# blasif/cocons

Measured on AMD Instinct MI355X. Metric: -2loglik evals/sec (dense cov_rns + Cholesky/solve/log-det, fp64) at n=10000, higher is better.
Workload: dtype f64

## Files before the change

### cocons_amd/csrc/chol.hip

```cpp
#include <hip/hip_runtime.h>
#include <limits.h>
#include <stdlib.h>
#include <string.h>
#include <algorithm>
#include <atomic>
#include <vector>
#include "kernels.h"

namespace cocons {

typedef double d4 __attribute__((ext_vector_type(4)));

#define MFMA64(a, b, c) __builtin_amdgcn_mfma_f64_16x16x4f64((a), (b), (c), 0, 0, 0)
#define MFMA64_NEGA(a, b, c) __builtin_amdgcn_mfma_f64_16x16x4f64((a), (b), (c), 0, 0, 1)
#define LDS_T __attribute__((address_space(3)))

__device__ __forceinline__ void blk_mma(d4 &acc, const d4 &P, const d4 &Q)
{
    acc = MFMA64(Q[0], P[0], acc);
    acc = MFMA64(Q[1], P[1], acc);
    acc = MFMA64(Q[2], P[2], acc);
    acc = MFMA64(Q[3], P[3], acc);
}

__device__ __forceinline__ d4 lds_blk(const double *blk, int lane)
{
    d4 v;
    int o = (lane >> 4) * 16 + (lane & 15);
    v[0] = blk[o];
    v[1] = blk[o + 64];
    v[2] = blk[o + 128];
    v[3] = blk[o + 192];
    return v;
}

__device__ __forceinline__ void lds_blk_store(double *blk, int lane, const d4 &v)
{
    int o = (lane >> 4) * 16 + (lane & 15);
    blk[o] = v[0];
    blk[o + 64] = v[1];
    blk[o + 128] = v[2];
    blk[o + 192] = v[3];
}

__device__ __forceinline__ d4 glb_blk(const double *A, size_t lda, int row0, int col0, int lane)
{
    const double *p = A + (size_t)(row0 + (lane & 15)) + (size_t)(col0 + (lane >> 4)) * lda;
    d4 v;
    v[0] = p[0];
    v[1] = p[4 * lda];
    v[2] = p[8 * lda];
    v[3] = p[12 * lda];
    return v;
}

__device__ __forceinline__ void glb_blk_store(double *A, size_t lda, int row0, int col0, int lane, const d4 &v)
{
    double *p = A + (size_t)(row0 + (lane & 15)) + (size_t)(col0 + (lane >> 4)) * lda;
    p[0] = v[0];
    p[4 * lda] = v[1];
    p[8 * lda] = v[2];
    p[12 * lda] = v[3];
}

__device__ __forceinline__ void store_wt(double *p, double v)
{
    __hip_atomic_store((unsigned long long *)p, (unsigned long long)__double_as_longlong(v), __ATOMIC_RELAXED,
                       __HIP_MEMORY_SCOPE_AGENT);
}

__device__ __forceinline__ double load_wt(const double *p)
{
    return __longlong_as_double((long long)__hip_atomic_load((const unsigned long long *)p, __ATOMIC_RELAXED,
                                                             __HIP_MEMORY_SCOPE_AGENT));
}

__device__ __forceinline__ d4 glb_blk_wt(const double *A, size_t lda, int row0, int col0, int lane)
{
    const double *p = A + (size_t)(row0 + (lane & 15)) + (size_t)(col0 + (lane >> 4)) * lda;
    d4 v;
    v[0] = load_wt(p);
    v[1] = load_wt(p + 4 * lda);
    v[2] = load_wt(p + 8 * lda);
    v[3] = load_wt(p + 12 * lda);
    return v;
}

__device__ __forceinline__ void glb_blk_store_wt(double *A, size_t lda, int row0, int col0, int lane, const d4 &v)
{
    double *p = A + (size_t)(row0 + (lane & 15)) + (size_t)(col0 + (lane >> 4)) * lda;
    store_wt(p, v[0]);
    store_wt(p + 4 * lda, v[1]);
    store_wt(p + 8 * lda, v[2]);
    store_wt(p + 12 * lda, v[3]);
}

__device__ __forceinline__ double rdlane(double v, int lane)
{
    int lo = __builtin_amdgcn_readlane(__double2loint(v), lane);
    int hi = __builtin_amdgcn_readlane(__double2hiint(v), lane);
    return __hiloint2double(hi, lo);
}

__device__ __forceinline__ void rsqrt_pivot(double a, double &l, double &r)
{
    const double y0 = __builtin_amdgcn_rsq(a);
    const double s0 = a * y0;
    const double t = fma(-s0, y0, 1.0);
    const double y = fma(y0 * t, fma(t, 0.375, 0.5), y0);
    double s = a * y;
    s = fma(fma(-s, s, a), 0.5 * y, s);
    l = s;
    r = y;
}

__device__ __forceinline__ double sel_lower4(int c, int k, double v00, double v10, double v11, double v20,
                                             double v21, double v22, double v30, double v31, double v32, double v33)
{
    double r0 = v00;
    double r1 = (k == 0) ? v10 : v11;
    double r2 = (k == 0) ? v20 : ((k == 1) ? v21 : v22);
    double r3 = (k == 0) ? v30 : ((k == 1) ? v31 : ((k == 2) ? v32 : v33));
    double r = (c == 0) ? r0 : ((c == 1) ? r1 : ((c == 2) ? r2 : r3));
    return (k <= c) ? r : 0.0;
}

template <int S>
__device__ __forceinline__ void potrf16_step(d4 &D, double (&Q)[4], int lane, int &fail)
{
    const int m = lane & 15, k = lane >> 4;
    const double ds = D[S];
    double a00 = rdlane(ds, 4 * S + 0), a10 = rdlane(ds, 4 * S + 1), a20 = rdlane(ds, 4 * S + 2),
           a30 = rdlane(ds, 4 * S + 3);
    double a11 = rdlane(ds, 4 * S + 1 + 16), a21 = rdlane(ds, 4 * S + 2 + 16), a31 = rdlane(ds, 4 * S + 3 + 16);
    double a22 = rdlane(ds, 4 * S + 2 + 32), a32 = rdlane(ds, 4 * S + 3 + 32);
    double a33 = rdlane(ds, 4 * S + 3 + 48);
    double l00, r0;
    rsqrt_pivot(a00, l00, r0);
    double l10 = a10 * r0, l20 = a20 * r0, l30 = a30 * r0;
    double t11 = fma(-l10, l10, a11);
    double l11, r1;
    rsqrt_pivot(t11, l11, r1);
    double l21 = fma(-l20, l10, a21) * r1, l31 = fma(-l30, l10, a31) * r1;
    double t22 = fma(-l21, l21, fma(-l20, l20, a22));
    double l22, r2;
    rsqrt_pivot(t22, l22, r2);
    double l32 = fma(-l31, l21, fma(-l30, l20, a32)) * r2;
    double t33 = fma(-l32, l32, fma(-l31, l31, fma(-l30, l30, a33)));
    double l33, r3;
    rsqrt_pivot(t33, l33, r3);
    if (__builtin_amdgcn_ballot_w64(!(t33 > 0.0)) != 0ull && fail == 0)
        fail = 4 * S + (!(a00 > 0.0) ? 1 : (!(t11 > 0.0) ? 2 : (!(t22 > 0.0) ? 3 : 4)));
    double m00 = r0, m11 = r1, m22 = r2, m33 = r3;
    double m10 = -(l10 * m00) * r1;
// ... 982 lines not shown
        }
    }
#pragma unroll
    for (int j = 0; j < 8; ++j) glb_blk_store(A, lda, rs, c0 + 16 * j, lane, B0[j]);
    if (split) return;
    if (tid == 0) ok = wait_ge<false>(xrw, 1u, abort_word, abort_code(ABORT_INPANEL, (unsigned)(c0 / TILE))) ? 1 : 0;
    asm volatile("s_waitcnt vmcnt(0)" ::: "memory");
    __syncthreads();
    if (!ok) return;
    {
        const int i = tid & 15, k = tid >> 4;
        const double *Xg = A + (size_t)(c1 + i) + (size_t)(c0 + k) * lda;
        double st[2][16];
#pragma unroll
        for (int b = 0; b < 16; ++b) st[0][b] = load_wt(Xg + (size_t)(16 * (b >> 3)) + (size_t)(16 * (b & 7)) * lda);
#pragma unroll
        for (int r = 0; r < 4; ++r) {
            if (r + 1 < 4) {
#pragma unroll
                for (int b = 0; b < 16; ++b) {
                    const int bb = 16 * (r + 1) + b;
                    st[(r + 1) & 1][b] = load_wt(Xg + (size_t)(16 * (bb >> 3)) + (size_t)(16 * (bb & 7)) * lda);
                }
            }
#pragma unroll
            for (int b = 0; b < 16; ++b) XS[(16 * r + b) * 256 + k * 16 + i] = st[r & 1][b];
        }
        __syncthreads();
#pragma unroll
        for (int jj = 0; jj < 8; ++jj) {
            d4 acc = {0.0, 0.0, 0.0, 0.0};
#pragma unroll
            for (int kb = 0; kb < 8; ++kb) {
                d4 Xb = lds_blk(XS + (jj * 8 + kb) * 256, lane);
                blk_mma(acc, B0[kb], Xb);
            }
            B1[jj] = B1[jj] - acc;
        }
    }
    __syncthreads();
    {
        const double *mb = mb1;
        double v9[3][9];
        MBOX_FETCH256V(0, v9[0])
        MBOX_FETCH256V(1, v9[1])
#pragma unroll
        for (int j = 0; j < 8; ++j) {
            double *LS = SM + (j & 1) * (9 * 256);
            MBOX_COMPLETE256V(j, v9[j % 3], abort_word, abort_code(ABORT_PANEL, (unsigned)(c1 / TILE)))
#pragma unroll
            for (int i = 0; i < 9; ++i)
                if (i <= 8 - j) LS[tid + 256 * i] = v9[j % 3][i];
            __syncthreads();
            if (!ok) return;
            if (j + 2 < 8) MBOX_FETCH256V(j + 2, v9[(j + 2) % 3])
            d4 L = lds_blk(LS, lane);
            double Q[4];
#pragma unroll
            for (int s = 0; s < 4; ++s) Q[s] = LS[(8 - j) * 256 + s * 64 + lane];
            trsm16(B1[j], L, Q);
            if (pub) mbox_store(sp + (size_t)(8 + j) * 1024, lane, B1[j]);
            d4 NX = -B1[j];
#pragma unroll
            for (int jj = j + 1; jj < 8; ++jj) {
                d4 Lb = lds_blk(LS + (jj - j) * 256, lane);
                blk_mma(B1[jj], NX, Lb);
            }
        }
    }
#pragma unroll
    for (int j = 0; j < 8; ++j) glb_blk_store(A, lda, rs, c1 + 16 * j, lane, B1[j]);
}

__global__ void __launch_bounds__(64)
engine_gate_kernel(unsigned *alive, unsigned *abort_word, unsigned code, unsigned long long ticks, unsigned nhelp,
                   unsigned *raise_in)
{
    if (threadIdx.x == 0) {
        bool ok = wait_ge<false>(alive, 1u, abort_word, code, ticks);
        if (ok && nhelp) ok = wait_ge<false>(alive + 2, nhelp, abort_word, code + 1u, ticks);
        if (ok && raise_in) {
            __hip_atomic_store(raise_in, 3u, __ATOMIC_RELAXED, __HIP_MEMORY_SCOPE_AGENT);
            __hip_atomic_store(raise_in + 1, 7u, __ATOMIC_RELAXED, __HIP_MEMORY_SCOPE_AGENT);
        }
    }
}

__global__ void __launch_bounds__(256)
trsm_tile_kernel(double *A, size_t lda, int c0, int r0, const double *qin, unsigned *wait_word, unsigned *abort_word,
                 int nb1, int e0, int own_world, int own_rank, int own_group)
{
    __shared__ double SL[36 * 256];
    __shared__ double QS[8 * 256];
    __shared__ int ok;
    const int tid = threadIdx.x, lane = tid & 63, wave = tid >> 6;
    if (own_world > 1) {
        const int row = (int)blockIdx.x < nb1 ? r0 + 64 * (int)blockIdx.x : e0 + 64 * ((int)blockIdx.x - nb1);
        if (((row / (2 * TILE) / own_group) % own_world) != own_rank) return;
    }
    if (wait_word) {
        if (tid == 0) ok = wait_ge<false>(wait_word, 1u, abort_word, abort_code(ABORT_PANEL, (unsigned)(c0 / TILE))) ? 1 : 0;
        asm volatile("s_waitcnt vmcnt(0)" ::: "memory");
        __syncthreads();
        if (!ok) return;
        fetch_factor_tile<true>(A, lda, c0, qin, SL, QS, tid);
    } else
        fetch_factor_tile<false>(A, lda, c0, qin, SL, QS, tid);
    const int bx = blockIdx.x;
    const int rs = (bx < nb1 ? r0 + 64 * bx : e0 + 64 * (bx - nb1)) + 16 * wave;
    d4 B[8];
#pragma unroll
    for (int j = 0; j < 8; ++j) B[j] = glb_blk(A, lda, rs, c0 + 16 * j, lane);
    __syncthreads();
#pragma unroll
    for (int j = 0; j < 8; ++j) {
        d4 L = lds_blk(SL + (j * (j + 1) / 2 + j) * 256, lane);
        double Q[4];
#pragma unroll
        for (int s = 0; s < 4; ++s) Q[s] = QS[j * 256 + s * 64 + lane];
        trsm16(B[j], L, Q);
        d4 NX = -B[j];
#pragma unroll
        for (int jj = j + 1; jj < 8; ++jj) {
            d4 Lb = lds_blk(SL + (jj * (jj + 1) / 2 + j) * 256, lane);
            blk_mma(B[jj], NX, Lb);
        }
    }
#pragma unroll
    for (int j = 0; j < 8; ++j) glb_blk_store(A, lda, rs, c0 + 16 * j, lane, B[j]);
}


struct UpdArgs {
    double *C; size_t ldc;
    const double *P; size_t ldp;
    int K;
    int ti0, tj0, lower_only;
    int H, W;
    unsigned *sig; int sig_tile;
    unsigned *wait_word, *abort_word;
    int ptiles, world, rank;
    const int *pmap;
    int skip_lo, skip_hi;
    unsigned *queue; unsigned ntiles;
    int Hb, ext0;
    int c_wt;
    int skew, kblk;
};

template <int TM, int KC, int ROLE, int NW = 4>
__global__ void __launch_bounds__(64 * NW, 8)
update_kernel(UpdArgs a)
{
    constexpr int LDT = TM + 16;
    constexpr int WY = NW / 2;
    constexpr int NB = TM / 32;
    constexpr int NBY = TM / WY / 16;
    constexpr int TPC = 64 * NW / KC;
    constexpr int RPT = TM / TPC;
    __shared__ double sI[2][KC * LDT];
    __shared__ double sJ[2][KC * LDT];
    unsigned *share = (unsigned *)&sI[0][TM];
    const int tid = threadIdx.x;
    const int wave_s = __builtin_amdgcn_readfirstlane(tid >> 6);
    if (a.wait_word) {
        if (tid == 0) *share = wait_ge(a.wait_word, 1u, a.abort_word, abort_code(ABORT_INPANEL, (unsigned)a.tj0)) ? 1u : 0u;
        asm volatile("s_waitcnt vmcnt(0)" ::: "memory");
        __syncthreads();
        const unsigned ok = *share;
        __syncthreads();
        if (!ok) return;
    }

    else if (a.abort_word) {
        if (tid == 0) *share = __hip_atomic_load(a.abort_word, __ATOMIC_RELAXED, __HIP_MEMORY_SCOPE_AGENT);
        __syncthreads();
        const unsigned ab = *share;
        __syncthreads();
        if (ab) return;
    }

    const int nch = a.K / KC;
    typedef double d2 __attribute__((ext_vector_type(2)));

    unsigned L = blockIdx.x;
    for (;;) {
        int lane;
        asm volatile("v_mbcnt_lo_u32_b32 %0, -1, 0\n\tv_mbcnt_hi_u32_b32 %0, -1, %0" : "=v"(lane));
        const int wave = wave_s, t2 = 64 * wave + lane;
        const int wi = wave & 1, wj = wave >> 1;
        const int kc = t2 / TPC, rg = (t2 % TPC) * RPT;
        const int ro = (lane >> 4) * LDT + (lane & 15);
        int ti, tj;
        if (a.lower_only) {
            int lo = 0, hi = a.W - 1;
            while (lo < hi) {
                const int mid = (lo + hi + 1) >> 1;
                if (mid * a.H - mid * (mid - 1) / 2 <= (int)L) lo = mid; else hi = mid - 1;
            }
            const int j = lo;
            const int til = j + ((int)L - (j * a.H - j * (j - 1) / 2));
            tj = a.tj0 + j;
            ti = til < a.Hb ? a.tj0 + til : a.ext0 + (til - a.Hb);
        } else {
            const int til = blockIdx.x;
            ti = til < a.Hb ? a.ti0 + til : a.ext0 + (til - a.Hb);
            tj = a.tj0 + blockIdx.y;
        }
        if (a.world > 1 && ((ti * TM / (2 * TILE) / a.ptiles) % a.world) != a.rank) return;
        if (ti >= a.skip_lo && ti < a.skip_hi && tj >= a.skip_lo && tj < a.skip_hi) {
            if (!a.queue) return;
            if (t2 == 0) *share = gridDim.x + __hip_atomic_fetch_add(a.queue, 1u, __ATOMIC_RELAXED, __HIP_MEMORY_SCOPE_AGENT);
            __syncthreads();
            L = (unsigned)__builtin_amdgcn_readfirstlane((int)*share);
            __syncthreads();
            if (L >= a.ntiles) break;
            continue;
        }
        const int sig_Ti = (ti * TM) / TILE - a.sig_tile, sig_Tj = (tj * TM) / TILE - a.sig_tile;
        const bool sig_wg = a.sig != nullptr && sig_Ti >= 0 && sig_Ti <= 1 && sig_Tj >= 0 && sig_Tj <= sig_Ti;
        const bool wt_wg = sig_wg || a.c_wt;
        if (sig_wg) __builtin_amdgcn_s_setprio(3); else __builtin_amdgcn_s_setprio(0);

        int rowI_P = ti * TM, rowJ_P = tj * TM, rowI_C = ti * TM;
        if (a.pmap) { rowI_P = a.pmap[ti]; rowJ_P = a.pmap[tj]; }
        if (a.skew) {
            const bool ext = ti >= a.ext0;
            const int under = a.skew * TILE + (ti - a.ext0) * TM;
            rowI_P = ext ? under : ti * TM - TILE * a.kblk;
            rowJ_P = tj * TM - TILE * a.kblk;
            rowI_C = ext ? under : ti * TM - TILE * ((tj * TM) / TILE);
        }
        const double *gI = a.P + (size_t)(rowI_P + rg) + (size_t)kc * a.ldp;
        const double *gJ = a.P + (size_t)(rowJ_P + rg) + (size_t)kc * a.ldp;
        d2 stI[RPT / 2], stJ[RPT / 2];

        double *Cb = a.C + (size_t)(rowI_C + (TM / 2) * wi) + (size_t)(tj * TM + (TM / WY) * wj) * a.ldc;
        const unsigned ldcb = 8u * (unsigned)a.ldc;
        const unsigned cvo = 8u * (unsigned)(lane & 15) + (unsigned)(lane >> 4) * ldcb;
        d4 acc[NB][NBY];
#pragma unroll
        for (int x = 0; x < NB; ++x)
#pragma unroll
            for (int y = 0; y < NBY; ++y) acc[x][y] = (d4){0.0, 0.0, 0.0, 0.0};

#pragma unroll
        for (int v = 0; v < RPT / 2; ++v) {
            stI[v] = *(const d2 *)(gI + 2 * v);
            stJ[v] = *(const d2 *)(gJ + 2 * v);
        }
#pragma unroll
        for (int v = 0; v < RPT / 2; ++v) {
            *(d2 *)(&sI[0][kc * LDT + rg + 2 * v]) = stI[v];
            *(d2 *)(&sJ[0][kc * LDT + rg + 2 * v]) = stJ[v];
        }
        __syncthreads();

        for (int ch = 0; ch < nch; ++ch) {
            const int cur = ch & 1;
            if (ch + 1 < nch) {
                const double *pI = gI + (size_t)(ch + 1) * KC * a.ldp;
                const double *pJ = gJ + (size_t)(ch + 1) * KC * a.ldp;
#pragma unroll
                for (int v = 0; v < RPT / 2; ++v) {
                    stI[v] = *(const d2 *)(pI + 2 * v);
                    stJ[v] = *(const d2 *)(pJ + 2 * v);
                }
            }
            const double *bI = &sI[cur][ro + (TM / 2) * wi];
            const double *bJ = &sJ[cur][ro + (TM / WY) * wj];
#pragma unroll
            for (int s = 0; s < KC / 4; ++s) {
                double pi_[NB], pj_[NBY];
#pragma unroll
                for (int x = 0; x < NB; ++x) pi_[x] = bI[s * 4 * LDT + 16 * x];
#pragma unroll
                for (int y = 0; y < NBY; ++y) pj_[y] = bJ[s * 4 * LDT + 16 * y];
#pragma unroll
                for (int x = 0; x < NB; ++x)
#pragma unroll
                    for (int y = 0; y < NBY; ++y) acc[x][y] = MFMA64(pj_[y], pi_[x], acc[x][y]);
            }
            if (ch + 1 < nch) {
#pragma unroll
                for (int v = 0; v < RPT / 2; ++v) {
                    *(d2 *)(&sI[cur ^ 1][kc * LDT + rg + 2 * v]) = stI[v];
                    *(d2 *)(&sJ[cur ^ 1][kc * LDT + rg + 2 * v]) = stJ[v];
                }
            }
            __syncthreads();
        }
        unsigned Lnext = 0;
        if (a.queue && t2 == 0)
            Lnext = gridDim.x + __hip_atomic_fetch_add(a.queue, 1u, __ATOMIC_RELAXED, __HIP_MEMORY_SCOPE_AGENT);
        unsigned cve = cvo;
        asm volatile("" : "+v"(cve));
#pragma unroll
        for (int x = 0; x < NB; ++x)
#pragma unroll
            for (int y = 0; y < NBY; ++y) {
                d4 cv;
#pragma unroll
                for (int r = 0; r < 4; ++r) {
                    const double *cp = (const double *)((const char *)(Cb + 16 * x) + (cve + (unsigned)(16 * y + 4 * r) * ldcb));
                    cv[r] = a.c_wt ? load_wt(cp) : *cp;
                }
                cv -= acc[x][y];
                if (wt_wg) {
#pragma unroll
                    for (int r = 0; r < 4; ++r)
                        store_wt((double *)((char *)(Cb + 16 * x) + (cve + (unsigned)(16 * y + 4 * r) * ldcb)), cv[r]);
                } else {
#pragma unroll
                    for (int r = 0; r < 4; ++r)
                        *(double *)((char *)(Cb + 16 * x) + (cve + (unsigned)(16 * y + 4 * r) * ldcb)) = cv[r];
                }
            }
        if (wt_wg) {
            asm volatile("s_waitcnt vmcnt(0)" ::: "memory");
            __syncthreads();
            if (t2 == 0 && sig_wg) signal_add(a.sig + a.sig_tile + sig_Ti);
        }
        if (!a.queue) break;
        if (t2 == 0) *share = Lnext;
        __syncthreads();
        L = (unsigned)__builtin_amdgcn_readfirstlane((int)*share);
        if (L >= a.ntiles) break;
    }
}

struct DagStep {
    unsigned base;
    unsigned near;
    unsigned tpos, nT;
    int H, W;
    int tj0;
    int k0, K;
    int nstrip, two;
    int need;
    int nd_next;
    int split;
    unsigned p2, p3;
};

struct DagArgs {
    double *A; size_t lda;
    double *P;
    const double *Wt;
    const DagStep *steps; int nsteps;
    unsigned ntasks;
    unsigned *queue;
    unsigned *tdone;
    unsigned *pdone; int pstride;
    unsigned *pall;
    double *partbuf;
    unsigned *dcount;
    unsigned *sig;
    unsigned *out, *xr;
    unsigned *abort_word;
    const unsigned *alive;
    unsigned xcc_quota;
    unsigned *hw;
    unsigned long long *trace;
    const unsigned *ftab;
    unsigned xcd_g;
    unsigned *xcnt;
};

constexpr unsigned DAG_XCD_LAG = 64u;
__device__ __forceinline__ unsigned dag_position(unsigned c, unsigned cls, unsigned g)
{
    return ((c >> g) << (g + 3u)) | (cls << g) | (c & ((1u << g) - 1u));
}

__device__ __forceinline__ bool dag_wait(const DagArgs &a, unsigned *word, unsigned need, unsigned code, unsigned L)
{
    const unsigned long long t0 = __builtin_amdgcn_s_memrealtime();
    for (unsigned it = 0;; ++it) {
        const unsigned v = poll_word(word, it);
        if (v >= need) break;
        if (__hip_atomic_load(a.abort_word, __ATOMIC_RELAXED, __HIP_MEMORY_SCOPE_AGENT) != 0u) return false;
        if (it > (unsigned)(ENGINE_TIMEOUT_TICKS / 100ull) ||
            ((it & 1023u) == 1023u && __builtin_amdgcn_s_memrealtime() - t0 > WALL_BACKSTOP_TICKS)) {
            if (__hip_atomic_exchange(a.abort_word, code, __ATOMIC_RELAXED, __HIP_MEMORY_SCOPE_AGENT) == 0u) {
                unsigned *d = a.queue + 8;
                d[0] = L; d[1] = code; d[2] = (unsigned)(word - a.queue); d[3] = need; d[4] = v;
                d[5] = (unsigned)(__builtin_amdgcn_s_memrealtime() - t0);
                d[6] = it;
            }
            return false;
        }
        __builtin_amdgcn_s_sleep(16);
    }
    __builtin_amdgcn_fence(__ATOMIC_ACQUIRE, "wavefront");
    return true;
}

__global__ void __launch_bounds__(256, 8)
dag_kernel(DagArgs a)
{
    constexpr int TM = 64, KC = 4, RING = 4, STG = 2 * KC * TM;
    __shared__ double smem[RING * STG + 2];
    unsigned *share = (unsigned *)&smem[RING * STG];
    const int tid = threadIdx.x;
    const int wave_s = __builtin_amdgcn_readfirstlane(tid >> 6);
    const DagStep *__restrict__ steps = a.steps;
    const unsigned ldab = 8u * (unsigned)a.lda;
    int known = 0;
    const unsigned myx = (hw_where() >> 28) & 7u;
    const bool loyal = ((blockIdx.x >> 3) & 1u) == 0u;
    if (tid == 0) {
        bool take = true;
        if (a.xcc_quota) {
            const unsigned c = __hip_atomic_load(a.alive + 16 + myx, __ATOMIC_RELAXED, __HIP_MEMORY_SCOPE_AGENT);
            if (c) {
                const unsigned less = 7u * (c - 1u);
                const unsigned quota = a.xcc_quota > less + 8u ? a.xcc_quota - less : 8u;
                take = __hip_atomic_fetch_add(a.queue + 16 + myx, 1u, __ATOMIC_RELAXED, __HIP_MEMORY_SCOPE_AGENT) < quota;
            }
        }
        unsigned first = 0xffffffffu;
        if (take) {
            if (a.xcd_g) first = dag_position(__hip_atomic_fetch_add(a.xcnt + 32u * myx, 1u, __ATOMIC_RELAXED, __HIP_MEMORY_SCOPE_AGENT), myx, a.xcd_g);
            else first = __hip_atomic_fetch_add(a.queue, 1u, __ATOMIC_RELAXED, __HIP_MEMORY_SCOPE_AGENT);
        }
        share[1] = first;
        share[2] = 0u;
    }
    __syncthreads();
    unsigned L = (unsigned)__builtin_amdgcn_readfirstlane((int)share[1]);
    __syncthreads();
    if (L >= a.ntasks) return;
    for (;;) {
        int lo = 0, hi = a.nsteps - 1;
        while (lo < hi) {
            const int mid = (lo + hi + 1) >> 1;
            if (steps[mid].base <= L) lo = mid; else hi = mid - 1;
        }
        const int s = lo;
        const DagStep st = steps[s];
        const unsigned q = L - st.base;
        if (a.trace && tid == 0) {
            a.trace[4 * (size_t)L] = __builtin_amdgcn_s_memrealtime();
            if (a.hw) a.hw[2 * (size_t)L] = hw_where();
// ... 497 lines not shown
__global__ void __launch_bounds__(256)
gather_rows_kernel(const double *Y, int ldy, const int *pos, int n, int ncol, double *out, int ldo)
{
    const int i = blockIdx.x * blockDim.x + threadIdx.x;
    if (i >= n) return;
    const int k = pos[i];
    for (int s = blockIdx.y; s < ncol; s += gridDim.y) out[(size_t)i + (size_t)s * ldo] = Y[(size_t)k + (size_t)s * ldy];
}

void launch_gather_rows(const double *Y, int ldy, const int *pos, int n, int ncol, double *out, int ldo, hipStream_t s)
{
    if (n <= 0 || ncol <= 0) return;
    const int gy = ncol < 64 ? ncol : 64;
    hipLaunchKernelGGL(gather_rows_kernel, dim3((n + 255) / 256, gy), dim3(256), 0, s, Y, ldy, pos, n, ncol, out, ldo);
}

static void set_dynamic_lds_once(const void *kernel, size_t bytes, std::atomic<unsigned long long> &done_mask)
{
    int dev = 0;
    (void)hipGetDevice(&dev);
    if (dev >= 0 && dev < 64 && ((done_mask.load(std::memory_order_relaxed) >> dev) & 1ull)) return;
    (void)hipFuncSetAttribute(kernel, hipFuncAttributeMaxDynamicSharedMemorySize, (int)bytes);
    if (dev >= 0 && dev < 64) done_mask.fetch_or(1ull << dev, std::memory_order_relaxed);
}

void launch_potrf_tile(double *A, size_t lda, int c0, double *dinv, int *info, hipStream_t s)
{
    const size_t shm = (36 + 1) * 256 * sizeof(double);
    static std::atomic<unsigned long long> attr_done{0};
    set_dynamic_lds_once((const void *)potrf_tile_kernel, shm, attr_done);
    hipLaunchKernelGGL(potrf_tile_kernel, dim3(1), dim3(512), shm, s, A, lda, c0, dinv, info);
}

__global__ void __launch_bounds__(64)
raise_word_kernel(unsigned *word)
{
    if (threadIdx.x == 0) __hip_atomic_store(word, 1u, __ATOMIC_RELAXED, __HIP_MEMORY_SCOPE_AGENT);
}

void launch_raise_word(unsigned *word, hipStream_t s) { hipLaunchKernelGGL(raise_word_kernel, dim3(1), dim3(64), 0, s, word); }

int streams_run_concurrently(hipStream_t first, hipStream_t second, unsigned *words)
{
    if (hipMemsetAsync(words, 0, 2 * sizeof(unsigned), second) != hipSuccess) return -1;
    if (hipStreamSynchronize(second) != hipSuccess) return -1;
    hipLaunchKernelGGL(engine_gate_kernel, dim3(1), dim3(64), 0, first, words, words + 1, 1u, 200000ull, 0u, (unsigned *)nullptr);
    hipLaunchKernelGGL(raise_word_kernel, dim3(1), dim3(64), 0, second, words);
    unsigned h[2] = {0, 0};
    if (hipStreamSynchronize(first) != hipSuccess || hipStreamSynchronize(second) != hipSuccess) return -1;
    if (hipMemcpyAsync(h, words, sizeof h, hipMemcpyDeviceToHost, second) != hipSuccess) return -1;
    if (hipStreamSynchronize(second) != hipSuccess) return -1;
    return h[1] == 0 ? 1 : 0;
}

void launch_engine_gate(unsigned *alive, unsigned *abort_word, hipStream_t s, bool last_tile, bool patient, int nhelp,
                        unsigned *raise_in)
{
    hipLaunchKernelGGL(engine_gate_kernel, dim3(1), dim3(64), 0, s, alive, abort_word, last_tile ? ABORT_LAST_TILE : ABORT_GATE,
                       last_tile ? ENGINE_TIMEOUT_TICKS : (patient ? 10 * GATE_TIMEOUT_TICKS : GATE_TIMEOUT_TICKS),
                       (unsigned)(last_tile || nhelp < 0 ? 0 : nhelp), last_tile ? nullptr : raise_in);
}

static size_t engine_lds_bytes()
{
    static size_t shm = 0;
    if (!shm) {
        shm = 150 * 1024;
        const char *x = getenv("COCONS_ENGINE_LDS");
        if (x && (size_t)atol(x) >= shm) shm = (size_t)atol(x);
    }
    return shm;
}

void launch_potrf_engine(double *A, size_t lda, int t0, int nt, double *dinv, int *info,
                         unsigned *in, unsigned *out, unsigned *xr, unsigned *abort_word, unsigned *alive, hipStream_t s,
                         double *wbuf, double *pbuf, int dag_until, unsigned long long *trace, double *mbox, int in_wait_ms)
{
    EngineArgs e;
    e.A = A; e.lda = lda; e.t0 = t0; e.nt = nt; e.dinv = dinv; e.info = info;
    e.in = in; e.out = out; e.xr = xr; e.abort_word = abort_word; e.alive = alive;
    e.wbuf = wbuf; e.pbuf = pbuf; e.dag_until = dag_until; e.trace = trace;
    e.in_ticks = in_wait_ms > 0 ? 100000ull * (unsigned long long)in_wait_ms : HOST_PACED_TICKS;
    e.mbox = mbox;
    e.partner = mbox ? 8 : 0;
    const int grid = e.partner ? e.partner + 1 : 1;
    const size_t shm = engine_lds_bytes();
    if (wbuf && pbuf) {
        static std::atomic<unsigned long long> attr_done{0};
        set_dynamic_lds_once((const void *)potrf_engine_kernel<true>, shm, attr_done);
        hipLaunchKernelGGL(potrf_engine_kernel<true>, dim3(grid), dim3(512), shm, s, e);
    } else {
        static std::atomic<unsigned long long> attr_done{0};
        set_dynamic_lds_once((const void *)potrf_engine_kernel<false>, shm, attr_done);
        hipLaunchKernelGGL(potrf_engine_kernel<false>, dim3(grid), dim3(512), shm, s, e);
    }
}

void launch_trsm_tile(double *A, size_t lda, int c0, int r0, int r1, const double *dinv, hipStream_t s,
                      unsigned *wait_word, unsigned *abort_word, int band_r1, int ext_r0, int own_world, int own_rank,
                      int own_group)
{
    int nb1 = ((band_r1 >= 0 ? band_r1 : r1) - r0) / 64, nb2 = band_r1 >= 0 ? (r1 - ext_r0) / 64 : 0;
    if (nb1 < 0) nb1 = 0;
    if (nb2 < 0) nb2 = 0;
    if (nb1 + nb2 <= 0) return;
    hipLaunchKernelGGL(trsm_tile_kernel, dim3(nb1 + nb2), dim3(256), 0, s, A, lda, c0, r0, dinv, wait_word, abort_word,
                       nb1, ext_r0, own_world, own_rank, own_group < 1 ? 1 : own_group);
}

void launch_potrf_follow(double *A, size_t lda, int c0, int r0, int r1, double *dinv, int *info, double *mbox,
                         unsigned *abort_word, hipStream_t s, int band_r1, int ext_r0)
{
    int nb1 = ((band_r1 >= 0 ? band_r1 : r1) - r0) / 64, nb2 = band_r1 >= 0 ? (r1 - ext_r0) / 64 : 0;
    if (nb1 < 0) nb1 = 0;
    if (nb2 < 0) nb2 = 0;
    const int nstrips = nb1 + nb2;
    static std::atomic<unsigned long long> attr_done{0};
    const size_t shm = 76 * 1024;
    set_dynamic_lds_once((const void *)potrf_follow_kernel, shm, attr_done);
    hipLaunchKernelGGL(potrf_follow_kernel, dim3(1 + (nstrips + 1) / 2), dim3(512), shm, s, A, lda, c0, dinv, info, mbox, r0, nb1,
                       ext_r0, nstrips, abort_word);
}

void launch_panel_pair(double *A, size_t lda, int c0, int r0, int r1, unsigned *xr, unsigned *abort_word, hipStream_t s,
                       const double *mb0, const double *mb1, double *smb, int ndiag, unsigned *sig, int sig_tile, double *xmb)
{
    const int nb = (r1 - r0) / 64;
    if (nb <= 0) return;
    const bool split = xmb != nullptr;
    const bool diag = smb && ndiag > 0 && nb >= (ndiag == 10 ? 4 : 2);
    hipLaunchKernelGGL(panel_pair_kernel, dim3((split ? 2 * nb : nb) + (diag ? ndiag : 0)), dim3(256), 0, s, A, lda, c0, r0,
                       xr, abort_word, mb0, mb1, diag ? smb : nullptr, nb, diag ? (ndiag == 10 ? 4 : 2) : 0, sig, sig_tile, xmb);
}

static int upd_waves = -1;
static long long upd_w8_max_tiles = -1;
void set_update_waves(int nw) { upd_waves = nw == 8 ? 8 : 4; }
void set_update_w8_max_tiles(int ntiles) { upd_w8_max_tiles = ntiles < 0 ? 0 : ntiles; }
static int upd_c_wt = 0;
void set_update_c_wt(int on) { upd_c_wt = on ? 1 : 0; }

void launch_update_from(double *A, size_t lda, const double *P, size_t ldp, int K,
                        int ti0, int ti1, int tj0, int tj1, bool lower_only, hipStream_t s,
                        int ptiles, int world, int rank, unsigned *sig, int sig_tile,
                        unsigned *wait_word, unsigned *abort_word, unsigned *queue, int band_hi, int ext0,
                        int skew, int kblk, int trim64, const int *pmap, int skip_lo, int skip_hi)
{
    const bool band = band_hi >= 0;
    const int rows_band = (band ? band_hi : ti1) - ti0, rows_ext = band ? ti1 - ext0 : 0;
    if (rows_band + rows_ext <= 0 || rows_band < 0 || rows_ext < 0 || tj1 <= tj0 || K <= 0) return;
    trim64 = trim64 ? 1 : 0;
    const int rows64 = 2 * (rows_band + rows_ext) - trim64;
    if (rows64 <= 0) return;
    if (upd_waves < 0) { const char *e = getenv("COCONS_UPD_WAVES"); set_update_waves(e ? atoi(e) : 8); }
    if (upd_w8_max_tiles < 0) { const char *e = getenv("COCONS_UPD_W8_MAX_TILES"); set_update_w8_max_tiles(e ? atoi(e) : 3500); }
    bool use_w8 = false;
    UpdArgs a;
    a.queue = nullptr; a.ntiles = 0;
    a.skew = skew; a.kblk = kblk; a.c_wt = upd_c_wt;
    a.Hb = 2 * rows_band; a.ext0 = 2 * ext0;
    a.C = A; a.ldc = lda; a.P = P; a.ldp = ldp; a.K = K;
    a.lower_only = lower_only ? 1 : 0;
    a.ptiles = ptiles < 1 ? 1 : ptiles; a.world = world; a.rank = rank; a.pmap = pmap; a.skip_lo = skip_lo; a.skip_hi = skip_hi;
    a.sig = sig; a.sig_tile = sig_tile;
    a.wait_word = wait_word; a.abort_word = abort_word;
    a.H = 0; a.W = 0;
    a.ti0 = 2 * ti0; a.tj0 = 2 * tj0;
    dim3 grid(rows64, 2 * (tj1 - tj0));
    if (lower_only) {
        if (ti0 != tj0) { a.lower_only = 0; }
        else {
            const long long H = rows64, W = 2LL * (tj1 - tj0);
            a.H = (int)H; a.W = (int)W;
            const long long total = W * H - W * (W - 1) / 2;
            static int slots = 0;
            if (!slots) {
                int dev = 0, cus = 256;
                hipGetDevice(&dev);
                hipDeviceGetAttribute(&cus, hipDeviceAttributeMultiprocessorCount, dev);
                slots = 8 * cus;
            }
            grid = dim3((unsigned)total, 1);
            if (queue && world == 1) {
                const bool w8 = upd_waves == 8 && K >= 2 * TILE && !skew &&
                                (upd_w8_max_tiles == 0 || total <= upd_w8_max_tiles);
                use_w8 = w8;
                const int cap = w8 ? slots / 2 - 4 : slots - 8;
                if (total > cap + (w8 ? 4 : 8)) {
                    a.queue = queue; a.ntiles = (unsigned)total;
                    grid = dim3((unsigned)cap, 1);
                }
            }
        }
    }
    const bool trailing = (K > TILE) && world == 1;
    if (trailing && use_w8 && a.lower_only) hipLaunchKernelGGL((update_kernel<64, 16, 0, 8>), grid, dim3(512), 0, s, a);
    else if (trailing) hipLaunchKernelGGL((update_kernel<64, 8, 0>), grid, dim3(256), 0, s, a);
    else hipLaunchKernelGGL((update_kernel<64, 8, 1>), grid, dim3(256), 0, s, a);
}

__global__ void __launch_bounds__(256)
pack_rows_kernel(const double *A, size_t lda, int col0, int ncols, double *dst, size_t ldp, const int *pmap, int ti_lo,
                 long long slot_lo, long long slot_hi)
{
    const int ti = ti_lo + (int)blockIdx.x;
    const long long off = pmap[ti];
    if (off < slot_lo || off >= slot_hi) return;
    const int rho = threadIdx.x & 63, cq = threadIdx.x >> 6;
    for (int c = 4 * (int)blockIdx.y + cq; c < ncols; c += 4 * (int)gridDim.y)
        dst[off + rho + (size_t)c * ldp] = A[(size_t)(64 * ti + rho) + (size_t)(col0 + c) * lda];
}

void launch_pack_rows(const double *A, size_t lda, int col0, int ncols, double *dst, size_t ldp, const int *pmap, int ti_lo,
                      int ti_hi, long long slot_lo, long long slot_hi, hipStream_t s)
{
    if (ti_hi <= ti_lo || ncols <= 0) return;
    hipLaunchKernelGGL(pack_rows_kernel, dim3(ti_hi - ti_lo, 8), dim3(256), 0, s, A, lda, col0, ncols, dst, ldp, pmap, ti_lo,
                       slot_lo, slot_hi);
}

static void dag_build_far_table(const std::vector<DagStepHost> &steps, std::vector<unsigned> &tab, int xcd_g, int bw, int bh)
{
    tab.assign(steps.size(), 0u);
    for (size_t s = 0; s < steps.size(); ++s) {
        const DagStepHost &st = steps[s];
        tab[s] = (unsigned)tab.size();
        const int nc = std::min(st.W, st.two ? 4 : 2);
        std::vector<std::vector<unsigned>> blocks;
        if (bw <= 0) {
            blocks.emplace_back();
            for (int jl = nc; jl < st.W; ++jl)
                for (int il = jl; il < st.H; ++il) blocks.back().push_back((unsigned)il << 16 | (unsigned)jl);
        } else {
            for (int c0 = nc; c0 < st.W; c0 += bw) {
                const int c1 = std::min(c0 + bw, st.W);
                for (int r0 = c0; r0 < st.H; r0 += bh) {
                    const int r1 = std::min(r0 + bh, st.H);
                    std::vector<unsigned> b;
                    for (int il = r0; il < r1; ++il)
                        for (int jl = c0; jl < c1 && jl <= il; ++jl) b.push_back((unsigned)il << 16 | (unsigned)jl);
                    if (!b.empty()) blocks.push_back(std::move(b));
                }
            }
        }
        const long long ntile = (long long)st.W * st.H - (long long)st.W * (st.W - 1) / 2;
        const long long nfar = ntile - st.near;
        const unsigned nA = 2u * (unsigned)st.nstrip + (unsigned)st.nd_next, perBC = st.two ? 2u * (unsigned)st.nstrip : 0u;
        const bool panels = st.nT > 0;
        size_t next_block = 0;
        size_t cur[8], pos_in[8];
        for (int x = 0; x < 8; ++x) { cur[x] = (size_t)-1; pos_in[x] = 0; }
        std::vector<size_t> taken_back(blocks.size(), 0);
        long long q = 0;
        const unsigned total = (unsigned)ntile + st.nT;
        for (unsigned pos = 0; pos < total && q < ntile; ++pos) {
            if (panels && ((pos >= st.tpos && pos < st.tpos + nA) || (pos >= st.p2 && pos < st.p2 + perBC) ||
                           (pos >= st.p3 && pos < st.p3 + perBC)))
                continue;
            const long long qt = q++;
            if (qt < (long long)st.near) continue;
            const int x = xcd_g > 0 ? (int)(((st.base + pos) >> xcd_g) & 7u) : 0;
            unsigned tile = 0;
            bool got = false;
            while (!got) {
                if (cur[x] != (size_t)-1 && pos_in[x] + taken_back[cur[x]] < blocks[cur[x]].size()) {
                    tile = blocks[cur[x]][pos_in[x]++];
                    got = true;
                } else if (next_block < blocks.size()) {
                    cur[x] = next_block++; pos_in[x] = 0;
                } else {
                    size_t best = (size_t)-1, left = 0;
                    for (int y = 0; y < 8; ++y)
                        if (cur[y] != (size_t)-1) {
                            const size_t l = blocks[cur[y]].size() - pos_in[y] - taken_back[cur[y]];
                            if (l > left) { left = l; best = cur[y]; }
                        }
                    if (best == (size_t)-1) break;
                    tile = blocks[best][blocks[best].size() - 1 - taken_back[best]++];
                    got = true;
                }
            }
            tab.push_back(tile);
        }
        (void)nfar;
    }
}

unsigned dag_build_steps(int nt, int mt, int trim64, int kskip, int lead, int min_tiles, std::vector<DagStepHost> &out,
                         int lead2, int lead3, std::vector<unsigned> *ftab, int xcd_g, int bw, int bh)
{
    out.clear();
    if (ftab) ftab->clear();
    unsigned base = 0;
    int prev_two = 1;
    for (int k = 0; k + 2 < nt; k += 2) {
        const int t = k + 2;
        {
            const long long H0 = 2LL * (mt - t) - (trim64 ? 1 : 0), W0 = 2LL * (nt - t);
            if (W0 * H0 - W0 * (W0 - 1) / 2 < min_tiles) break;
        }
        DagStepHost st;
        st.tj0 = 2 * t;
        st.H = 2 * (mt - t) - (trim64 ? 1 : 0);
        st.W = 2 * (nt - t);
        st.two = t + 1 < nt ? 1 : 0;
        const long long tiles = (long long)st.W * st.H - (long long)st.W * (st.W - 1) / 2;
        const int nc = std::min(st.W, st.two ? 4 : 2);
        st.near = (unsigned)(nc * st.H - nc * (nc - 1) / 2);
        st.nstrip = std::max(0, st.H - (st.two ? 4 : 2));
        st.nT = (unsigned)(st.nstrip * (st.two ? 6 : 2));
        st.k0 = k * TILE + (k == 0 ? kskip : 0);
        st.K = 2 * TILE - (k == 0 ? kskip : 0);
        st.need = prev_two ? 6 : 2;
        st.nd_next = 0; st.split = 0;
        st.tpos = 0; st.p2 = 0; st.p3 = 0;
        st.base = 0;
        prev_two = st.two;
        (void)tiles;
        out.push_back(st);
    }
    if (!out.empty()) {
        DagStepHost &l = out.back();
        l.nT = 0; l.nstrip = 0;
    }
    for (size_t s = 0; s + 1 < out.size(); ++s)
        if (out[s].nstrip > 0 && out[s].two) {
            out[s].nd_next = out[s + 1].two ? 10 : 3;
            out[s + 1].split = 1;
        }
    for (auto &st : out) {
        const long long ntile = (long long)st.W * st.H - (long long)st.W * (st.W - 1) / 2;
        st.nT += (unsigned)st.nd_next;
        const long long nA = 2LL * st.nstrip + st.nd_next;
        const long long perBC = st.two ? 2LL * st.nstrip : 0;
        const long long far = ntile - st.near;
        st.tpos = st.near + (unsigned)std::min<long long>(far, lead);
        st.base = base;
// ... 254 lines not shown
```

Measured before the change: 125.7.

## Stream update-kernel operands via global_load_lds into a 4-stage LDS ring

Replaces the register-staged double-buffered copy of panel operands in the trailing-update kernel with direct global-to-LDS DMA loads (global_load_lds) into a four-slot ring, using a swizzled layout instead of padding. Each stage is waited on with vmcnt counters and a single barrier, so loads run up to three chunks ahead of the MFMA work. The goal is to cut VGPR staging traffic and per-chunk synchronisation and to hide global latency better. It adds alignment and K-divisibility requirements, enforced by a host-side check that reports an error and launches an empty kernel when they are not met.

```diff
diff --git a/cocons_amd/csrc/chol.hip b/cocons_amd/csrc/chol.hip
--- a/cocons_amd/csrc/chol.hip
+++ b/cocons_amd/csrc/chol.hip
@@ -1,5 +1,7 @@
 #include <hip/hip_runtime.h>
 #include <limits.h>
+#include <stdint.h>
+#include <stdio.h>
 #include <stdlib.h>
 #include <string.h>
 #include <algorithm>
@@ -1288,15 +1290,13 @@
 __global__ void __launch_bounds__(64 * NW, 8)
 update_kernel(UpdArgs a)
 {
-    constexpr int LDT = TM + 16;
+    static_assert(TM == 64 && KC == 2 * NW, "a wave's DMA fills two 64-row columns: NW columns per operand and stage");
     constexpr int WY = NW / 2;
     constexpr int NB = TM / 32;
     constexpr int NBY = TM / WY / 16;
-    constexpr int TPC = 64 * NW / KC;
-    constexpr int RPT = TM / TPC;
-    __shared__ double sI[2][KC * LDT];
-    __shared__ double sJ[2][KC * LDT];
-    unsigned *share = (unsigned *)&sI[0][TM];
+    constexpr int SC = KC / 2, RING = 4, STG = 2 * SC * TM;
+    __shared__ double smem[RING * STG + 2];
+    unsigned *share = (unsigned *)&smem[RING * STG];
     const int tid = threadIdx.x;
     const int wave_s = __builtin_amdgcn_readfirstlane(tid >> 6);
     if (a.wait_word) {
@@ -1316,8 +1316,7 @@
         if (ab) return;
     }
 
-    const int nch = a.K / KC;
-    typedef double d2 __attribute__((ext_vector_type(2)));
+    const int nch = a.K / SC;
 
     unsigned L = blockIdx.x;
     for (;;) {
@@ -1325,8 +1324,6 @@
         asm volatile("v_mbcnt_lo_u32_b32 %0, -1, 0\n\tv_mbcnt_hi_u32_b32 %0, -1, %0" : "=v"(lane));
         const int wave = wave_s, t2 = 64 * wave + lane;
         const int wi = wave & 1, wj = wave >> 1;
-        const int kc = t2 / TPC, rg = (t2 % TPC) * RPT;
-        const int ro = (lane >> 4) * LDT + (lane & 15);
         int ti, tj;
         if (a.lower_only) {
             int lo = 0, hi = a.W - 1;
@@ -1367,10 +1364,6 @@
             rowJ_P = tj * TM - TILE * a.kblk;
             rowI_C = ext ? under : ti * TM - TILE * ((tj * TM) / TILE);
         }
-        const double *gI = a.P + (size_t)(rowI_P + rg) + (size_t)kc * a.ldp;
-        const double *gJ = a.P + (size_t)(rowJ_P + rg) + (size_t)kc * a.ldp;
-        d2 stI[RPT / 2], stJ[RPT / 2];
-
         double *Cb = a.C + (size_t)(rowI_C + (TM / 2) * wi) + (size_t)(tj * TM + (TM / WY) * wj) * a.ldc;
         const unsigned ldcb = 8u * (unsigned)a.ldc;
         const unsigned cvo = 8u * (unsigned)(lane & 15) + (unsigned)(lane >> 4) * ldcb;
@@ -1380,52 +1373,54 @@
 #pragma unroll
             for (int y = 0; y < NBY; ++y) acc[x][y] = (d4){0.0, 0.0, 0.0, 0.0};
 
-#pragma unroll
-        for (int v = 0; v < RPT / 2; ++v) {
-            stI[v] = *(const d2 *)(gI + 2 * v);
-            stJ[v] = *(const d2 *)(gJ + 2 * v);
-        }
-#pragma unroll
-        for (int v = 0; v < RPT / 2; ++v) {
-            *(d2 *)(&sI[0][kc * LDT + rg + 2 * v]) = stI[v];
-            *(d2 *)(&sJ[0][kc * LDT + rg + 2 * v]) = stJ[v];
-        }
-        __syncthreads();
-
-        for (int ch = 0; ch < nch; ++ch) {
-            const int cur = ch & 1;
-            if (ch + 1 < nch) {
-                const double *pI = gI + (size_t)(ch + 1) * KC * a.ldp;
-                const double *pJ = gJ + (size_t)(ch + 1) * KC * a.ldp;
-#pragma unroll
-                for (int v = 0; v < RPT / 2; ++v) {
-                    stI[v] = *(const d2 *)(pI + 2 * v);
-                    stJ[v] = *(const d2 *)(pJ + 2 * v);
-                }
-            }
-            const double *bI = &sI[cur][ro + (TM / 2) * wi];
-            const double *bJ = &sJ[cur][ro + (TM / WY) * wj];
-#pragma unroll
-            for (int s = 0; s < KC / 4; ++s) {
-                double pi_[NB], pj_[NBY];
-#pragma unroll
-                for (int x = 0; x < NB; ++x) pi_[x] = bI[s * 4 * LDT + 16 * x];
-#pragma unroll
-                for (int y = 0; y < NBY; ++y) pj_[y] = bJ[s * 4 * LDT + 16 * y];
-#pragma unroll
-                for (int x = 0; x < NB; ++x)
-#pragma unroll
-                    for (int y = 0; y < NBY; ++y) acc[x][y] = MFMA64(pj_[y], pi_[x], acc[x][y]);
-            }
-            if (ch + 1 < nch) {
-#pragma unroll
-                for (int v = 0; v < RPT / 2; ++v) {
-                    *(d2 *)(&sI[cur ^ 1][kc * LDT + rg + 2 * v]) = stI[v];
-                    *(d2 *)(&sJ[cur ^ 1][kc * LDT + rg + 2 * v]) = stJ[v];
-                }
-            }
-            __syncthreads();
-        }
+        const bool opJ = wave >= NW / 2;
+        const unsigned ldg = 8u * (unsigned)a.ldp, cstep = (unsigned)SC * ldg;
+        const int sc = (lane >> 5) & 1;
+        const char *src = (const char *)(a.P + (size_t)(opJ ? rowJ_P : rowI_P)) +
+                          ((unsigned)(2 * (wave & (NW / 2 - 1)) + sc) * ldg + 8u * (unsigned)((2 * (lane & 31)) ^ (16 * sc)));
+        LDS_T double *ldst = (LDS_T double *)(smem + 128 * wave);
+#define UPD_STAGE(slot)                                                                                                     \
+        do {                                                                                                                \
+            __builtin_amdgcn_global_load_lds((const void *)src, (LDS_T void *)(ldst + STG * (slot)), 16, 0, 0);            \
+            src += cstep;                                                                                                   \
+        } while (0)
+        const int kq = lane >> 4, kodd = kq & 1, rl = (lane & 15) + TM * kq;
+        int aI[NB], aJ[NBY];
+#pragma unroll
+        for (int x = 0; x < NB; ++x) aI[x] = rl + (((TM / 2) * wi + 16 * x) ^ (16 * kodd));
+#pragma unroll
+        for (int y = 0; y < NBY; ++y) aJ[y] = SC * TM + rl + (((TM / WY) * wj + 16 * y) ^ (16 * kodd));
+        UPD_STAGE(0);
+        if (nch > 1) UPD_STAGE(1);
+        if (nch > 2) UPD_STAGE(2);
+        for (int c0 = 0; c0 < nch; c0 += RING) {
+#pragma unroll
+            for (int r = 0; r < RING; ++r) {
+                const int ch = c0 + r;
+                if (r > 0 && ch >= nch) break;
+                if (ch + 2 < nch) asm volatile("s_waitcnt vmcnt(2)" ::: "memory");
+                else if (ch + 1 < nch) asm volatile("s_waitcnt vmcnt(1)" ::: "memory");
+                else asm volatile("s_waitcnt vmcnt(0)" ::: "memory");
+                asm volatile("s_waitcnt lgkmcnt(0)" ::: "memory");
+                __builtin_amdgcn_s_barrier();
+                asm volatile("" ::: "memory");
+                if (ch + RING - 1 < nch) UPD_STAGE((r + RING - 1) % RING);
+                const double *bs = smem + STG * r;
+#pragma unroll
+                for (int s = 0; s < SC / 4; ++s) {
+                    double pi_[NB], pj_[NBY];
+#pragma unroll
+                    for (int x = 0; x < NB; ++x) pi_[x] = bs[s * 4 * TM + aI[x]];
+#pragma unroll
+                    for (int y = 0; y < NBY; ++y) pj_[y] = bs[s * 4 * TM + aJ[y]];
+#pragma unroll
+                    for (int x = 0; x < NB; ++x)
+#pragma unroll
+                        for (int y = 0; y < NBY; ++y) acc[x][y] = MFMA64(pj_[y], pi_[x], acc[x][y]);
+                }
+            }
+        }
+#undef UPD_STAGE
         unsigned Lnext = 0;
         if (a.queue && t2 == 0)
             Lnext = gridDim.x + __hip_atomic_fetch_add(a.queue, 1u, __ATOMIC_RELAXED, __HIP_MEMORY_SCOPE_AGENT);
@@ -2229,6 +2224,12 @@
     trim64 = trim64 ? 1 : 0;
     const int rows64 = 2 * (rows_band + rows_ext) - trim64;
     if (rows64 <= 0) return;
+    if (K % 4 != 0 || ((uintptr_t)P & 15u) != 0 || ldp % 2 != 0 || ldp >= ((size_t)1 << 25)) {
+        fprintf(stderr, "launch_update_from: K = %d, P = %p, ldp = %zu: K must be a multiple of 4, P 16-byte aligned, ldp even\n",
+                K, (const void *)P, ldp);
+        hipLaunchKernelGGL((update_kernel<64, 8, 1>), dim3(1), dim3(0), 0, s, UpdArgs{});
+        return;
+    }
     if (upd_waves < 0) { const char *e = getenv("COCONS_UPD_WAVES"); set_update_waves(e ? atoi(e) : 8); }
     if (upd_w8_max_tiles < 0) { const char *e = getenv("COCONS_UPD_W8_MAX_TILES"); set_update_w8_max_tiles(e ? atoi(e) : 3500); }
     bool use_w8 = false;
@@ -2259,7 +2260,7 @@
             }
             grid = dim3((unsigned)total, 1);
             if (queue && world == 1) {
-                const bool w8 = upd_waves == 8 && K >= 2 * TILE && !skew &&
+                const bool w8 = upd_waves == 8 && K >= 2 * TILE && K % 8 == 0 && !skew &&
                                 (upd_w8_max_tiles == 0 || total <= upd_w8_max_tiles);
                 use_w8 = w8;
                 const int cap = w8 ? slots / 2 - 4 : slots - 8;
```

Result: no change. 125.4 (-0.2%).
